# BillyXYB/TransEditor

Hardware: AMD Instinct MI355X
Metric: 256x256 images/sec/GPU, G+D fwd+bwd, batch 16; 1/2/4/8-GPU scaling (higher is better)
Workload: dtype f32

## Files before the change

### transeditor_amd/csrc/rgb.hip

```cpp
#include "te_common.h"

namespace {

constexpr int KMAX = 512;
constexpr int NOUT = 3;

__global__ __launch_bounds__(256) void rgb_fwd_kernel(float* __restrict__ out, const float* __restrict__ x,
                                                      const float* __restrict__ w, const float* __restrict__ isc,
                                                      const float* __restrict__ bias, float wscale, int K, int HW) {
    __shared__ float ws[NOUT][KMAX];
    const int b = blockIdx.y, tid = threadIdx.x;
    for (int k = tid; k < K; k += 256) {
        const float s = (isc ? isc[(size_t)b * K + k] : 1.f) * wscale;
#pragma unroll
        for (int o = 0; o < NOUT; ++o) ws[o][k] = w[o * K + k] * s;
    }
    __syncthreads();
    const int HW4 = HW >> 2;
    const int p4 = blockIdx.x * 256 + tid;
    if (p4 >= HW4) return;
    const float4* xp = reinterpret_cast<const float4*>(x + (size_t)b * K * HW) + p4;
    float4 acc[NOUT];
#pragma unroll
    for (int o = 0; o < NOUT; ++o) acc[o] = make_float4(0.f, 0.f, 0.f, 0.f);
#pragma unroll 8
    for (int k = 0; k < K; ++k) {
        const float4 v = xp[(size_t)k * HW4];
#pragma unroll
        for (int o = 0; o < NOUT; ++o) {
            const float c = ws[o][k];
            acc[o].x += c * v.x; acc[o].y += c * v.y; acc[o].z += c * v.z; acc[o].w += c * v.w;
        }
    }
#pragma unroll
    for (int o = 0; o < NOUT; ++o) {
        const float bb = bias ? bias[o] : 0.f;
        acc[o].x += bb; acc[o].y += bb; acc[o].z += bb; acc[o].w += bb;
        reinterpret_cast<float4*>(out + ((size_t)b * NOUT + o) * HW)[p4] = acc[o];
    }
}

__global__ __launch_bounds__(256) void rgb_dgrad_kernel(float* __restrict__ gx, const float* __restrict__ g,
                                                        const float* __restrict__ w, const float* __restrict__ isc,
                                                        float wscale, int K, int HW, const float* __restrict__ bias = nullptr,
                                                        int act = 0) {
    __shared__ float ws[NOUT][KMAX];
    const int b = blockIdx.y, tid = threadIdx.x;
    for (int k = tid; k < K; k += 256) {
        const float s = (isc ? isc[(size_t)b * K + k] : 1.f) * wscale;
#pragma unroll
        for (int o = 0; o < NOUT; ++o) ws[o][k] = w[o * K + k] * s;
    }
    __syncthreads();
    const int HW4 = HW >> 2;
    const int p4 = blockIdx.x * 256 + tid;
    if (p4 >= HW4) return;
    float4 gv[NOUT];
#pragma unroll
    for (int o = 0; o < NOUT; ++o) gv[o] = reinterpret_cast<const float4*>(g + ((size_t)b * NOUT + o) * HW)[p4];
    float4* op = reinterpret_cast<float4*>(gx + (size_t)b * K * HW) + p4;
    const float gain = act == 3 ? 1.4142135623730951f : 1.f;
#pragma unroll 4
    for (int k = 0; k < K; ++k) {
        const float c0 = ws[0][k], c1 = ws[1][k], c2 = ws[2][k];
        const float bb = bias ? bias[k] : 0.f;
        float4 r;
        r.x = c0 * gv[0].x + c1 * gv[1].x + c2 * gv[2].x + bb;
        r.y = c0 * gv[0].y + c1 * gv[1].y + c2 * gv[2].y + bb;
        r.z = c0 * gv[0].z + c1 * gv[1].z + c2 * gv[2].z + bb;
        r.w = c0 * gv[0].w + c1 * gv[1].w + c2 * gv[2].w + bb;
        if (act >= 3) {
            r.x = (r.x > 0.f ? r.x : 0.2f * r.x) * gain; r.y = (r.y > 0.f ? r.y : 0.2f * r.y) * gain;
            r.z = (r.z > 0.f ? r.z : 0.2f * r.z) * gain; r.w = (r.w > 0.f ? r.w : 0.2f * r.w) * gain;
        }
        op[(size_t)k * HW4] = r;
    }
}

inline int rgb_pow2(int v) { int p = 1; while (p < v) p <<= 1; return p; }
inline int rgb_tile_px(int K) { return std::max(32, std::min(256, 8192 / rgb_pow2(K))); }

template <bool SUM>
__global__ __launch_bounds__(256) void rgb_wgrad_kernel(float* __restrict__ slabs, const float* __restrict__ g,
                                                        const float* __restrict__ x, int K, int HW, int S, int TPX, int lgTPX, int K2) {
    constexpr int NROW = SUM ? NOUT + 1 : NOUT;
    extern __shared__ __attribute__((aligned(16))) float smem[];
    float* xl = smem;
    float* gl = smem + K * (TPX + 1);
    const int b = blockIdx.y, c = blockIdx.x, tid = threadIdx.x;
    const int ntile = (HW + TPX - 1) / TPX;
    const int t0 = (int)((int64_t)ntile * c / S), t1 = (int)((int64_t)ntile * (c + 1) / S);
    const float* xb = x + (size_t)b * K * HW;
    const float* gb = g + (size_t)b * NOUT * HW;
    const bool vec4 = (HW & 3) == 0 && ((reinterpret_cast<uintptr_t>(x) & 15) == 0);
    const int parts = K2 >= 256 ? 1 : 256 / K2;
    const int kk = K2 >= 256 ? tid : (tid & (K2 - 1)), part = K2 >= 256 ? 0 : tid / K2;
    const int nh = K2 > 256 ? 2 : 1;
    float acc[2][NOUT + 1] = {{0.f, 0.f, 0.f, 0.f}, {0.f, 0.f, 0.f, 0.f}};
    for (int tl = t0; tl < t1; ++tl) {
        const int p0 = tl * TPX;
        __syncthreads();
        if (vec4) {
            for (int e0 = 0; e0 < K * TPX; e0 += 256 * 8 * 4) {
                float4 st[8];
#pragma unroll
                for (int j = 0; j < 8; ++j) {
                    const int e = e0 + 4 * (tid + 256 * j), k = e >> lgTPX, pp = e & (TPX - 1);
                    const bool ok = e < K * TPX && p0 + pp < HW;
                    st[j] = ok ? *reinterpret_cast<const float4*>(xb + (size_t)k * HW + p0 + pp) : make_float4(0.f, 0.f, 0.f, 0.f);
                }
#pragma unroll
                for (int j = 0; j < 8; ++j) {
                    const int e = e0 + 4 * (tid + 256 * j), k = e >> lgTPX, pp = e & (TPX - 1);
                    if (e < K * TPX) {
                        float* d = xl + k * (TPX + 1) + pp;
                        d[0] = st[j].x; d[1] = st[j].y; d[2] = st[j].z; d[3] = st[j].w;
                    }
                }
            }
        } else {
            for (int e0 = 0; e0 < K * TPX; e0 += 256 * 8) {
                float st[8];
#pragma unroll
                for (int j = 0; j < 8; ++j) {
                    const int e = e0 + tid + 256 * j, k = e >> lgTPX, pp = e & (TPX - 1);
                    const bool ok = e < K * TPX && p0 + pp < HW;
                    const float v = xb[ok ? (size_t)k * HW + p0 + pp : 0];
                    st[j] = ok ? v : 0.f;
                }
#pragma unroll
                for (int j = 0; j < 8; ++j) {
                    const int e = e0 + tid + 256 * j, k = e >> lgTPX, pp = e & (TPX - 1);
                    if (e < K * TPX) xl[k * (TPX + 1) + pp] = st[j];
                }
            }
        }
        for (int e = tid; e < NOUT * TPX; e += 256) {
            const int o = e >> lgTPX, pp = e & (TPX - 1);
            gl[e] = (p0 + pp < HW) ? gb[(size_t)o * HW + p0 + pp] : 0.f;
        }
        __syncthreads();
        for (int h = 0; h < nh; ++h) {
            const int k = kk + 256 * h;
            if (k < K) {
#pragma unroll 4
                for (int pp = part; pp < TPX; pp += parts) {
                    const float xv = xl[k * (TPX + 1) + pp];
#pragma unroll
                    for (int o = 0; o < NOUT; ++o) acc[h][o] += gl[o * TPX + pp] * xv;
                    if (SUM) acc[h][NOUT] += xv;
                }
            }
        }
    }
    float* sl = slabs + ((size_t)b * S + c) * NROW * K;
    if (parts > 1) {
        __syncthreads();
        float* red = smem;
#pragma unroll
        for (int o = 0; o < NROW; ++o) red[(part * NROW + o) * K2 + kk] = acc[0][o];
        __syncthreads();
        if (part == 0 && kk < K) {
#pragma unroll
            for (int o = 0; o < NROW; ++o) {
                float a = 0.f;
                for (int q = 0; q < parts; ++q) a += red[(q * NROW + o) * K2 + kk];
                sl[o * K + kk] = a;
            }
        }
        return;
    }
    for (int h = 0; h < nh; ++h) {
        const int k = kk + 256 * h;
        if (k < K) {
#pragma unroll
            for (int o = 0; o < NROW; ++o) sl[o * K + k] = acc[h][o];
        }
    }
}

inline bool ok_shape(int K, int HW) { return K > 0 && K <= KMAX && HW > 0 && (HW & 3) == 0; }

}

extern "C" int te_rgb_supported(int M, int K, int HW) { return (M == NOUT && ok_shape(K, HW)) ? 1 : 0; }

extern "C" int te_rgb_fwd_f32(float* out, const float* x, const float* w, const float* isc, const float* bias, float wscale,
                              int B, int K, int HW, te_stream_t stream_) {
    TE_REQUIRE(out && x && w, TE_ERR_NULL, "te_rgb_fwd_f32: NULL pointer");
    TE_REQUIRE(B > 0 && ok_shape(K, HW), TE_ERR_UNSUPPORTED, "te_rgb_fwd_f32: need K <= 512 and H*W %% 4 == 0");
    dim3 grid((unsigned)te::cdiv(HW / 4, 256), (unsigned)B);
    rgb_fwd_kernel<<<grid, 256, 0, (hipStream_t)stream_>>>(out, x, w, isc, bias, wscale, K, HW);
    return te::launch_status("te_rgb_fwd_f32");
}

extern "C" int te_rgb_dgrad_f32(float* gx, const float* g, const float* w, const float* isc, float wscale, int B, int K,
                                int HW, te_stream_t stream_) {
    TE_REQUIRE(gx && g && w, TE_ERR_NULL, "te_rgb_dgrad_f32: NULL pointer");
    TE_REQUIRE(B > 0 && ok_shape(K, HW), TE_ERR_UNSUPPORTED, "te_rgb_dgrad_f32: need K <= 512 and H*W %% 4 == 0");
    dim3 grid((unsigned)te::cdiv(HW / 4, 256), (unsigned)B);
    rgb_dgrad_kernel<<<grid, 256, 0, (hipStream_t)stream_>>>(gx, g, w, isc, wscale, K, HW);
    return te::launch_status("te_rgb_dgrad_f32");
}

extern "C" int te_rgb_expand_f32(float* out, const float* x3, const float* w, const float* bias, int act, float wscale, int B,
                                 int K, int HW, te_stream_t stream_) {
    TE_REQUIRE(out && x3 && w, TE_ERR_NULL, "te_rgb_expand_f32: NULL pointer");
    TE_REQUIRE(B > 0 && ok_shape(K, HW), TE_ERR_UNSUPPORTED, "te_rgb_expand_f32: need K <= 512 and H*W %% 4 == 0");
    TE_REQUIRE(act == 0 || act == 3 || act == 4, TE_ERR_UNSUPPORTED, "te_rgb_expand_f32: act must be 0, 3 or 4");
    dim3 grid((unsigned)te::cdiv(HW / 4, 256), (unsigned)B);
    rgb_dgrad_kernel<<<grid, 256, 0, (hipStream_t)stream_>>>(out, x3, w, nullptr, wscale, K, HW, bias, act);
    return te::launch_status("te_rgb_expand_f32");
}

extern "C" int te_rgb_wgrad_slab_count(int B, int K, int HW) {
    if (B <= 0 || K <= 0 || HW <= 0) return TE_ERR_SHAPE;
    const int64_t ntile = te::cdiv(HW, rgb_tile_px(K));
    int64_t S = te::cdiv(4 * te::kNumCU, B);
    return (int)std::max<int64_t>(1, std::min<int64_t>(S, ntile));
}

extern "C" int te_rgb_wgrad_f32(float* slabs, const float* g, const float* x, int B, int K, int HW, int S, te_stream_t stream_) {
    TE_REQUIRE(slabs && g && x, TE_ERR_NULL, "te_rgb_wgrad_f32: NULL pointer");
    TE_REQUIRE(B > 0 && K > 0 && K <= KMAX && HW > 0 && S > 0, TE_ERR_UNSUPPORTED, "te_rgb_wgrad_f32: need 0 < K <= 512");
    const int TPX = rgb_tile_px(K), K2 = rgb_pow2(K);
    int lg = 0;
    while ((1 << lg) < TPX) ++lg;
    const size_t lds = sizeof(float) * std::max<size_t>((size_t)K * (TPX + 1) + NOUT * TPX, (size_t)256 * (NOUT + 1));
    static std::atomic<uint64_t> attr_done{0};
    te::allow_big_lds(attr_done, (const void*)rgb_wgrad_kernel<false>, 96 * 1024);
    dim3 grid((unsigned)S, (unsigned)B);
    rgb_wgrad_kernel<false><<<grid, 256, lds, (hipStream_t)stream_>>>(slabs, g, x, K, HW, S, TPX, lg, K2);
    return te::launch_status("te_rgb_wgrad_f32");
}

extern "C" int te_rgb_wgrad_sum_f32(float* slabs, const float* g, const float* x, int B, int K, int HW, int S, te_stream_t stream_) {
    TE_REQUIRE(slabs && g && x, TE_ERR_NULL, "te_rgb_wgrad_sum_f32: NULL pointer");
    TE_REQUIRE(B > 0 && K > 0 && K <= KMAX && HW > 0 && S > 0, TE_ERR_UNSUPPORTED, "te_rgb_wgrad_sum_f32: need 0 < K <= 512");
    const int TPX = rgb_tile_px(K), K2 = rgb_pow2(K);
    int lg = 0;
    while ((1 << lg) < TPX) ++lg;
    const size_t lds = sizeof(float) * std::max<size_t>((size_t)K * (TPX + 1) + NOUT * TPX, (size_t)256 * (NOUT + 1));
    static std::atomic<uint64_t> attr_done{0};
    te::allow_big_lds(attr_done, (const void*)rgb_wgrad_kernel<true>, 96 * 1024);
    dim3 grid((unsigned)S, (unsigned)B);
    rgb_wgrad_kernel<true><<<grid, 256, lds, (hipStream_t)stream_>>>(slabs, g, x, K, HW, S, TPX, lg, K2);
    return te::launch_status("te_rgb_wgrad_sum_f32");
}
```

Measured before the change: 150.9.

## Add small-plane ToRGB kernels and software-pipeline the weight-gradient tile loads

Adds specialised forward and dgrad/expand kernels for small spatial planes where the old per-pixel grid left most CUs idle. The forward variant stages x in LDS and splits output channels across threads, and the dgrad variant spreads K×HW work across blocks. The wgrad kernel now prefetches the next tile into registers while it multiplies the current one, and is templated on register depth with launch-bounds occupancy hints. This adds code paths and register pressure, and uses clamped loads for out-of-range rows.

```diff
diff --git a/transeditor_amd/csrc/rgb.hip b/transeditor_amd/csrc/rgb.hip
--- a/transeditor_amd/csrc/rgb.hip
+++ b/transeditor_amd/csrc/rgb.hip
@@ -77,11 +77,99 @@
     }
 }
 
+constexpr int RGB_SMALL_LGQ_MAX = 3;
+
+template <int R>
+__global__ __launch_bounds__(256) void rgb_fwd_small_kernel(float* __restrict__ out, const float* __restrict__ x,
+                                                            const float* __restrict__ w, const float* __restrict__ isc,
+                                                            const float* __restrict__ bias, float wscale, int K, int HW, int lgQ) {
+    __shared__ float ws[NOUT][KMAX];
+    extern __shared__ __attribute__((aligned(16))) float smem[];
+    float4* xs = reinterpret_cast<float4*>(smem);
+    const int b = blockIdx.y, tid = threadIdx.x;
+    const int Q = 1 << lgQ, HW4 = HW >> 2, q0 = blockIdx.x * Q, nq = min(Q, HW4 - q0), n = K * Q;
+    const float4* xp = reinterpret_cast<const float4*>(x + (size_t)b * K * HW) + q0;
+    float4 st[R];
+#pragma unroll
+    for (int j = 0; j < R; ++j) {
+        const int e = min(tid + 256 * j, n - 1), k = e >> lgQ, q = min(e & (Q - 1), nq - 1);
+        st[j] = xp[(size_t)k * HW4 + q];
+    }
+#pragma unroll
+    for (int j = 0; j < R; ++j) xs[tid + 256 * j] = st[j];
+    for (int k = tid; k < K; k += 256) {
+        const float s = (isc ? isc[(size_t)b * K + k] : 1.f) * wscale;
+#pragma unroll
+        for (int o = 0; o < NOUT; ++o) ws[o][k] = w[o * K + k] * s;
+    }
+    __syncthreads();
+    const int o = tid >> (lgQ + 2), r = tid & (4 * Q - 1), q = r >> 2;
+    if (o >= NOUT || q >= nq) return;
+    const float* xf = smem + r;
+    float acc = 0.f;
+#pragma unroll 8
+    for (int k = 0; k < K; ++k) {
+        const float c = ws[o][k];
+        acc += c * xf[(size_t)k * 4 * Q];
+    }
+    const float bb = bias ? bias[o] : 0.f;
+    acc += bb;
+    out[((size_t)b * NOUT + o) * HW + 4 * q0 + r] = acc;
+}
+
+template <int R>
+void rgb_fwd_small_launch(dim3 grid, hipStream_t stream, float* out, const float* x, const float* w, const float* isc,
+                          const float* bias, float wscale, int K, int HW, int lgQ) {
+    static std::atomic<uint64_t> attr_done{0};
+    te::allow_big_lds(attr_done, (const void*)rgb_fwd_small_kernel<R>, 256 * R * (int)sizeof(float4));
+    rgb_fwd_small_kernel<R><<<grid, 256, 256 * R * sizeof(float4), stream>>>(out, x, w, isc, bias, wscale, K, HW, lgQ);
+}
+
+constexpr int RGB_SMALL_EPT = 4;
+
+__global__ __launch_bounds__(256) void rgb_dgrad_small_kernel(float* __restrict__ gx, const float* __restrict__ g,
+                                                              const float* __restrict__ w, const float* __restrict__ isc,
+                                                              float wscale, int K, int HW, const float* __restrict__ bias, int act) {
+    const int b = blockIdx.y, HW4 = HW >> 2;
+    const unsigned n = (unsigned)K * (unsigned)HW4;
+    const float4* gp = reinterpret_cast<const float4*>(g + (size_t)b * NOUT * HW);
+    float4* op = reinterpret_cast<float4*>(gx + (size_t)b * K * HW);
+    const float gain = act == 3 ? 1.4142135623730951f : 1.f;
+#pragma unroll
+    for (int j = 0; j < RGB_SMALL_EPT; ++j) {
+        const unsigned i = (blockIdx.x * RGB_SMALL_EPT + j) * 256u + threadIdx.x;
+        if (i >= n) break;
+        const unsigned k = i / (unsigned)HW4, p4 = i - k * (unsigned)HW4;
+        const float s = (isc ? isc[(size_t)b * K + k] : 1.f) * wscale;
+        const float c0 = w[k] * s, c1 = w[K + k] * s, c2 = w[2 * K + k] * s;
+        const float4 g0 = gp[p4], g1 = gp[HW4 + p4], g2 = gp[2 * HW4 + p4];
+        const float bb = bias ? bias[k] : 0.f;
+        float4 r;
+        r.x = c0 * g0.x + c1 * g1.x + c2 * g2.x + bb;
+        r.y = c0 * g0.y + c1 * g1.y + c2 * g2.y + bb;
+        r.z = c0 * g0.z + c1 * g1.z + c2 * g2.z + bb;
+        r.w = c0 * g0.w + c1 * g1.w + c2 * g2.w + bb;
+        if (act >= 3) {
+            r.x = (r.x > 0.f ? r.x : 0.2f * r.x) * gain; r.y = (r.y > 0.f ? r.y : 0.2f * r.y) * gain;
+            r.z = (r.z > 0.f ? r.z : 0.2f * r.z) * gain; r.w = (r.w > 0.f ? r.w : 0.2f * r.w) * gain;
+        }
+        op[i] = r;
+    }
+}
+
+inline bool rgb_small_plane(int B, int HW) { return HW <= 4096 && te::cdiv(HW / 4, 256) * B < te::kNumCU; }
+inline bool rgb_small_plane_fwd(int B, int HW) { return rgb_small_plane(B, HW) && (int64_t)HW * B <= 32768; }
+inline int rgb_small_lgq(int B, int HW) {
+    int lg = RGB_SMALL_LGQ_MAX;
+    while (lg > 0 && te::cdiv(HW / 4, 1 << lg) * B < 2 * te::kNumCU) --lg;
+    return lg;
+}
+
 inline int rgb_pow2(int v) { int p = 1; while (p < v) p <<= 1; return p; }
 inline int rgb_tile_px(int K) { return std::max(32, std::min(256, 8192 / rgb_pow2(K))); }
 
-template <bool SUM>
-__global__ __launch_bounds__(256) void rgb_wgrad_kernel(float* __restrict__ slabs, const float* __restrict__ g,
+template <bool SUM, int NP>
+__global__ __launch_bounds__(256, NP == 8 ? 4 : 2) void rgb_wgrad_kernel(float* __restrict__ slabs, const float* __restrict__ g,
                                                         const float* __restrict__ x, int K, int HW, int S, int TPX, int lgTPX, int K2) {
     constexpr int NROW = SUM ? NOUT + 1 : NOUT;
     extern __shared__ __attribute__((aligned(16))) float smem[];
@@ -92,55 +180,13 @@
     const int t0 = (int)((int64_t)ntile * c / S), t1 = (int)((int64_t)ntile * (c + 1) / S);
     const float* xb = x + (size_t)b * K * HW;
     const float* gb = g + (size_t)b * NOUT * HW;
-    const bool vec4 = (HW & 3) == 0 && ((reinterpret_cast<uintptr_t>(x) & 15) == 0);
+    const bool vec4 = (HW & 3) == 0 && ((reinterpret_cast<uintptr_t>(x) & 15) == 0) && (int64_t)K * HW < (1 << 30);
     const int parts = K2 >= 256 ? 1 : 256 / K2;
     const int kk = K2 >= 256 ? tid : (tid & (K2 - 1)), part = K2 >= 256 ? 0 : tid / K2;
-    const int nh = K2 > 256 ? 2 : 1;
-    float acc[2][NOUT + 1] = {{0.f, 0.f, 0.f, 0.f}, {0.f, 0.f, 0.f, 0.f}};
-    for (int tl = t0; tl < t1; ++tl) {
-        const int p0 = tl * TPX;
-        __syncthreads();
-        if (vec4) {
-            for (int e0 = 0; e0 < K * TPX; e0 += 256 * 8 * 4) {
-                float4 st[8];
-#pragma unroll
-                for (int j = 0; j < 8; ++j) {
-                    const int e = e0 + 4 * (tid + 256 * j), k = e >> lgTPX, pp = e & (TPX - 1);
-                    const bool ok = e < K * TPX && p0 + pp < HW;
-                    st[j] = ok ? *reinterpret_cast<const float4*>(xb + (size_t)k * HW + p0 + pp) : make_float4(0.f, 0.f, 0.f, 0.f);
-                }
-#pragma unroll
-                for (int j = 0; j < 8; ++j) {
-                    const int e = e0 + 4 * (tid + 256 * j), k = e >> lgTPX, pp = e & (TPX - 1);
-                    if (e < K * TPX) {
-                        float* d = xl + k * (TPX + 1) + pp;
-                        d[0] = st[j].x; d[1] = st[j].y; d[2] = st[j].z; d[3] = st[j].w;
-                    }
-                }
-            }
-        } else {
-            for (int e0 = 0; e0 < K * TPX; e0 += 256 * 8) {
-                float st[8];
-#pragma unroll
-                for (int j = 0; j < 8; ++j) {
-                    const int e = e0 + tid + 256 * j, k = e >> lgTPX, pp = e & (TPX - 1);
-                    const bool ok = e < K * TPX && p0 + pp < HW;
-                    const float v = xb[ok ? (size_t)k * HW + p0 + pp : 0];
-                    st[j] = ok ? v : 0.f;
-                }
-#pragma unroll
-                for (int j = 0; j < 8; ++j) {
-                    const int e = e0 + tid + 256 * j, k = e >> lgTPX, pp = e & (TPX - 1);
-                    if (e < K * TPX) xl[k * (TPX + 1) + pp] = st[j];
-                }
-            }
-        }
-        for (int e = tid; e < NOUT * TPX; e += 256) {
-            const int o = e >> lgTPX, pp = e & (TPX - 1);
-            gl[e] = (p0 + pp < HW) ? gb[(size_t)o * HW + p0 + pp] : 0.f;
-        }
-        __syncthreads();
-        for (int h = 0; h < nh; ++h) {
+    constexpr int NH = NP > 8 ? 2 : 1;
+    float acc[NH][NOUT + 1] = {};
+    auto multiply = [&]() {
+        for (int h = 0; h < NH; ++h) {
             const int k = kk + 256 * h;
             if (k < K) {
 #pragma unroll 4
@@ -152,6 +198,83 @@
                 }
             }
         }
+    };
+    if (vec4) {
+        const int pp0 = (4 * tid) & (TPX - 1), k0 = (4 * tid) >> lgTPX, kstep = 1024 >> lgTPX;
+        const unsigned lane_off = (unsigned)k0 * (unsigned)HW + (unsigned)pp0;
+        float* const lane_dst = xl + k0 * (TPX + 1) + pp0;
+        float4 st[NP];
+        float gr[NOUT];
+        auto fetch8 = [&](int p0, int j0) {
+            const bool col = p0 + pp0 < HW;
+#pragma unroll
+            for (int j = 0; j < 8; ++j) {
+                const int kj = (j0 + j) * kstep;
+                const float* base = xb + (size_t)min(kj, K - 1) * HW + p0;
+                st[j0 + j] = *reinterpret_cast<const float4*>(base + (col && k0 + kj < K ? lane_off : 0u));
+            }
+        };
+        auto fetch = [&](int p0) {
+            fetch8(p0, 0);
+            if (NP > 8) fetch8(p0, 8);
+#pragma unroll
+            for (int i = 0; i < NOUT; ++i) {
+                const int e = tid + 256 * i, o = e >> lgTPX, pp = e & (TPX - 1);
+                gr[i] = gb[e < NOUT * TPX && p0 + pp < HW ? (size_t)o * HW + p0 + pp : 0];
+            }
+        };
+        auto stash8 = [&](int p0, int j0) {
+            const bool col = p0 + pp0 < HW;
+#pragma unroll
+            for (int j = 0; j < 8; ++j) {
+                const int kj = (j0 + j) * kstep;
+                if (k0 + kj < K) {
+                    float* d = lane_dst + kj * (TPX + 1);
+                    const float4 v = st[j0 + j];
+                    d[0] = col ? v.x : 0.f; d[1] = col ? v.y : 0.f; d[2] = col ? v.z : 0.f; d[3] = col ? v.w : 0.f;
+                }
+            }
+        };
+        if (t0 < t1) fetch(t0 * TPX);
+        for (int tl = t0; tl < t1; ++tl) {
+            const int p0 = tl * TPX;
+            __syncthreads();
+            stash8(p0, 0);
+            if (NP > 8) stash8(p0, 8);
+#pragma unroll
+            for (int i = 0; i < NOUT; ++i) {
+                const int e = tid + 256 * i, pp = e & (TPX - 1);
+                if (e < NOUT * TPX) gl[e] = p0 + pp < HW ? gr[i] : 0.f;
+            }
+            __syncthreads();
+            if (tl + 1 < t1) fetch(p0 + TPX);
+            multiply();
+        }
+    }
+    for (int tl = vec4 ? t1 : t0; tl < t1; ++tl) {
+        const int p0 = tl * TPX;
+        __syncthreads();
+        for (int e0 = 0; e0 < K * TPX; e0 += 256 * 8) {
+            float st[8];
+#pragma unroll
+            for (int j = 0; j < 8; ++j) {
+                const int e = e0 + tid + 256 * j, k = e >> lgTPX, pp = e & (TPX - 1);
+                const bool ok = e < K * TPX && p0 + pp < HW;
+                const float v = xb[ok ? (size_t)k * HW + p0 + pp : 0];
+                st[j] = ok ? v : 0.f;
+            }
+#pragma unroll
+            for (int j = 0; j < 8; ++j) {
+                const int e = e0 + tid + 256 * j, k = e >> lgTPX, pp = e & (TPX - 1);
+                if (e < K * TPX) xl[k * (TPX + 1) + pp] = st[j];
+            }
+        }
+        for (int e = tid; e < NOUT * TPX; e += 256) {
+            const int o = e >> lgTPX, pp = e & (TPX - 1);
+            gl[e] = (p0 + pp < HW) ? gb[(size_t)o * HW + p0 + pp] : 0.f;
+        }
+        __syncthreads();
+        multiply();
     }
     float* sl = slabs + ((size_t)b * S + c) * NROW * K;
     if (parts > 1) {
@@ -170,12 +293,26 @@
         }
         return;
     }
-    for (int h = 0; h < nh; ++h) {
+    for (int h = 0; h < NH; ++h) {
         const int k = kk + 256 * h;
         if (k < K) {
 #pragma unroll
             for (int o = 0; o < NROW; ++o) sl[o * K + k] = acc[h][o];
         }
+    }
+}
+
+template <bool SUM>
+void rgb_wgrad_launch(size_t lds, float* slabs, const float* g, const float* x, int B, int K, int HW, int S, int TPX, int lg, int K2,
+                      hipStream_t stream) {
+    static std::atomic<uint64_t> attr_done8{0}, attr_done16{0};
+    dim3 grid((unsigned)S, (unsigned)B);
+    if (K <= 256) {
+        te::allow_big_lds(attr_done8, (const void*)rgb_wgrad_kernel<SUM, 8>, 96 * 1024);
+        rgb_wgrad_kernel<SUM, 8><<<grid, 256, lds, stream>>>(slabs, g, x, K, HW, S, TPX, lg, K2);
+    } else {
+        te::allow_big_lds(attr_done16, (const void*)rgb_wgrad_kernel<SUM, 16>, 96 * 1024);
+        rgb_wgrad_kernel<SUM, 16><<<grid, 256, lds, stream>>>(slabs, g, x, K, HW, S, TPX, lg, K2);
     }
 }
 
@@ -189,17 +326,40 @@
                               int B, int K, int HW, te_stream_t stream_) {
     TE_REQUIRE(out && x && w, TE_ERR_NULL, "te_rgb_fwd_f32: NULL pointer");
     TE_REQUIRE(B > 0 && ok_shape(K, HW), TE_ERR_UNSUPPORTED, "te_rgb_fwd_f32: need K <= 512 and H*W %% 4 == 0");
+    if (rgb_small_plane_fwd(B, HW)) {
+        const int lgQ = rgb_small_lgq(B, HW), rounds = (int)te::cdiv((int64_t)K << lgQ, 256);
+        dim3 grid((unsigned)te::cdiv(HW / 4, 1 << lgQ), (unsigned)B);
+        hipStream_t st = (hipStream_t)stream_;
+        if (rounds <= 1) rgb_fwd_small_launch<1>(grid, st, out, x, w, isc, bias, wscale, K, HW, lgQ);
+        else if (rounds <= 2) rgb_fwd_small_launch<2>(grid, st, out, x, w, isc, bias, wscale, K, HW, lgQ);
+        else if (rounds <= 4) rgb_fwd_small_launch<4>(grid, st, out, x, w, isc, bias, wscale, K, HW, lgQ);
+        else if (rounds <= 8) rgb_fwd_small_launch<8>(grid, st, out, x, w, isc, bias, wscale, K, HW, lgQ);
+        else rgb_fwd_small_launch<16>(grid, st, out, x, w, isc, bias, wscale, K, HW, lgQ);
+        return te::launch_status("te_rgb_fwd_f32");
+    }
     dim3 grid((unsigned)te::cdiv(HW / 4, 256), (unsigned)B);
     rgb_fwd_kernel<<<grid, 256, 0, (hipStream_t)stream_>>>(out, x, w, isc, bias, wscale, K, HW);
     return te::launch_status("te_rgb_fwd_f32");
+}
+
+namespace {
+void rgb_dgrad_launch(float* gx, const float* g, const float* w, const float* isc, float wscale, int B, int K, int HW,
+                      const float* bias, int act, hipStream_t stream) {
+    if (rgb_small_plane(B, HW)) {
+        dim3 grid((unsigned)te::cdiv((int64_t)K * (HW / 4), 256 * RGB_SMALL_EPT), (unsigned)B);
+        rgb_dgrad_small_kernel<<<grid, 256, 0, stream>>>(gx, g, w, isc, wscale, K, HW, bias, act);
+        return;
+    }
+    dim3 grid((unsigned)te::cdiv(HW / 4, 256), (unsigned)B);
+    rgb_dgrad_kernel<<<grid, 256, 0, stream>>>(gx, g, w, isc, wscale, K, HW, bias, act);
+}
 }
 
 extern "C" int te_rgb_dgrad_f32(float* gx, const float* g, const float* w, const float* isc, float wscale, int B, int K,
                                 int HW, te_stream_t stream_) {
     TE_REQUIRE(gx && g && w, TE_ERR_NULL, "te_rgb_dgrad_f32: NULL pointer");
     TE_REQUIRE(B > 0 && ok_shape(K, HW), TE_ERR_UNSUPPORTED, "te_rgb_dgrad_f32: need K <= 512 and H*W %% 4 == 0");
-    dim3 grid((unsigned)te::cdiv(HW / 4, 256), (unsigned)B);
-    rgb_dgrad_kernel<<<grid, 256, 0, (hipStream_t)stream_>>>(gx, g, w, isc, wscale, K, HW);
+    rgb_dgrad_launch(gx, g, w, isc, wscale, B, K, HW, nullptr, 0, (hipStream_t)stream_);
     return te::launch_status("te_rgb_dgrad_f32");
 }
 
@@ -208,8 +368,7 @@
     TE_REQUIRE(out && x3 && w, TE_ERR_NULL, "te_rgb_expand_f32: NULL pointer");
     TE_REQUIRE(B > 0 && ok_shape(K, HW), TE_ERR_UNSUPPORTED, "te_rgb_expand_f32: need K <= 512 and H*W %% 4 == 0");
     TE_REQUIRE(act == 0 || act == 3 || act == 4, TE_ERR_UNSUPPORTED, "te_rgb_expand_f32: act must be 0, 3 or 4");
-    dim3 grid((unsigned)te::cdiv(HW / 4, 256), (unsigned)B);
-    rgb_dgrad_kernel<<<grid, 256, 0, (hipStream_t)stream_>>>(out, x3, w, nullptr, wscale, K, HW, bias, act);
+    rgb_dgrad_launch(out, x3, w, nullptr, wscale, B, K, HW, bias, act, (hipStream_t)stream_);
     return te::launch_status("te_rgb_expand_f32");
 }
 
@@ -227,10 +386,7 @@
     int lg = 0;
     while ((1 << lg) < TPX) ++lg;
     const size_t lds = sizeof(float) * std::max<size_t>((size_t)K * (TPX + 1) + NOUT * TPX, (size_t)256 * (NOUT + 1));
-    static std::atomic<uint64_t> attr_done{0};
-    te::allow_big_lds(attr_done, (const void*)rgb_wgrad_kernel<false>, 96 * 1024);
-    dim3 grid((unsigned)S, (unsigned)B);
-    rgb_wgrad_kernel<false><<<grid, 256, lds, (hipStream_t)stream_>>>(slabs, g, x, K, HW, S, TPX, lg, K2);
+    rgb_wgrad_launch<false>(lds, slabs, g, x, B, K, HW, S, TPX, lg, K2, (hipStream_t)stream_);
     return te::launch_status("te_rgb_wgrad_f32");
 }
 
@@ -241,9 +397,6 @@
     int lg = 0;
     while ((1 << lg) < TPX) ++lg;
     const size_t lds = sizeof(float) * std::max<size_t>((size_t)K * (TPX + 1) + NOUT * TPX, (size_t)256 * (NOUT + 1));
-    static std::atomic<uint64_t> attr_done{0};
-    te::allow_big_lds(attr_done, (const void*)rgb_wgrad_kernel<true>, 96 * 1024);
-    dim3 grid((unsigned)S, (unsigned)B);
-    rgb_wgrad_kernel<true><<<grid, 256, lds, (hipStream_t)stream_>>>(slabs, g, x, K, HW, S, TPX, lg, K2);
+    rgb_wgrad_launch<true>(lds, slabs, g, x, B, K, HW, S, TPX, lg, K2, (hipStream_t)stream_);
     return te::launch_status("te_rgb_wgrad_sum_f32");
 }
```

New measurement: 152.2 (median of 6 runs). No clear change (+0.8%).
